# wangchou/whisper.coreml

Hardware: AMD Instinct MI355X
Metric: xRT (audio-s/s) large-v3 beam=5 @1/2/4/8 GPU; p50 per-token decode ms (higher is better)
Workload: dtype fp16; 1 GPU; large-v3 beam=5 transcribe() of one 600 s file, 30 s clip grid, condition_on_previous_text=False, temperature=0; model=large-v3, global_batch=20, seq_len=448

## Files before the change

include/whisper_hip.h:

```cpp
#ifndef WHISPER_HIP_H
#define WHISPER_HIP_H
#include <stdint.h>

#ifdef __cplusplus
extern "C" {
#endif

typedef struct wh_ctx wh_ctx;

typedef struct wh_dims {
  int n_mels, n_audio_ctx, n_audio_state, n_audio_head, n_audio_layer;
  int n_vocab, n_text_ctx, n_text_state, n_text_head, n_text_layer;
} wh_dims;

enum { WH_F32 = 0, WH_F16 = 1 };

typedef struct wh_decode_opts {
  int group;
  int beam;
  float patience;
  float temperature;
  int sample_len;
  int suppress_blank;
  int timestamps;
// ... 63 lines not shown
int wh_decode_maxc(wh_ctx* ctx);

int wh_prefill(wh_ctx* ctx, int n_win, int group, const int* tokens, const int* n_tokens, int max_tokens,
               const int* sot_index, float* logits);
int wh_step(wh_ctx* ctx, const int* tokens, const int* text_offsets, float* logits);
int wh_reorder_kv(wh_ctx* ctx, const int* source_rows);

int wh_prefill_logits(wh_ctx* ctx, int slot, const int* tokens, int n_tokens, float* logits, const int* align_heads,
                      int n_align, float* align_qk);

int wh_align(wh_ctx* ctx, int slot, const int* tokens, int n_tokens, int n_sot, int num_frames, const int* align_heads,
             int n_align, int medfilt_width, float* token_probs, int* path, int* path_len);
int wh_align_batch(wh_ctx* ctx, int n_win, const int* slots, const int* tokens, const int* n_tokens, int n_sot,
                   const int* num_frames, const int* align_heads, int n_align, int medfilt_width, float* token_probs,
                   int* paths, int* path_lens);
int wh_dtw(wh_ctx* ctx, const float* x, int n_rows, int n_cols, int* path, int* path_len);

int wh_step_kernels(wh_ctx* ctx, int n_win, int group, char* buf, int cap);

enum { WH_N_STATS = 16 };
enum {
  WH_STAT_MEL_MS = 0, WH_STAT_ENCODE_MS, WH_STAT_PREFILL_MS, WH_STAT_STEPS_MS, WH_STAT_STEPS, WH_STAT_ENCODE_WINDOWS,
  WH_STAT_INGEST_COPY_MS, WH_STAT_INGEST_KERNEL_MS, WH_STAT_FLAC_UPLOAD_MS, WH_STAT_FLAC_PARSE_MS,
  WH_STAT_FLAC_RESTORE_MS, WH_STAT_FLAC_GATHER_MS, WH_STAT_FLAC_RESAMPLE_MS, WH_STAT_FLAC_INDEX_MS,
  WH_STAT_VAD_ENERGY_MS, WH_STAT_VAD_SPANS_MS
};
int wh_stats(wh_ctx* ctx, double* out, int n);
int wh_sync(wh_ctx* ctx);

int wh_token_ms(wh_ctx* ctx, float* out, int cap, int* n, int reset);

int wh_time_stage(wh_ctx* ctx, int what, int iters, double* ms_per_iter);

int wh_flac_info(const uint8_t* data, int64_t n, int* sample_rate, int* channels, int* bits_per_sample,
                 int64_t* total_samples);
int wh_flac_decode(const uint8_t* data, int64_t n, int32_t* out, int64_t cap_frames, int64_t* n_frames);
const char* wh_flac_last_error(void);

int wh_flac_index(const uint8_t* data, int64_t n, int64_t* offsets, int32_t* fields, int64_t cap, int64_t* n_cand);
int wh_flac_decode_indexed(const uint8_t* data, int64_t n, int32_t* out, int64_t cap_frames, int64_t* n_frames);
int wh_flac_last_path(void);
int wh_flac_decode_device(wh_ctx* ctx, const uint8_t* data, int64_t n_bytes, int32_t* out, int64_t cap_frames,
                          int64_t* n_frames, int* path_out);
int wh_flac_ingest(wh_ctx* ctx, const uint8_t* data, int64_t n_bytes, int up, int down, const double* taps,
                   int n_taps, int64_t dst_offset, int64_t reserve, int64_t* n_out, int* path_out);

enum { WH_WAV_U8 = 0, WH_WAV_S16, WH_WAV_S24, WH_WAV_S32, WH_WAV_F32, WH_WAV_F64, WH_WAV_ALAW, WH_WAV_ULAW };
typedef struct wh_wav_fmt { int encoding, channels, sample_rate, valid_bits; int64_t data_offset, n_frames; } wh_wav_fmt;
int wh_wav_info(const uint8_t* data, int64_t n, wh_wav_fmt* out);
const char* wh_wav_last_error(void);
int wh_wav_ingest(wh_ctx* ctx, const uint8_t* data, int64_t n_bytes, int up, int down, const double* taps,
                  int n_taps, int64_t dst_offset, int64_t reserve, int64_t* n_out);

#ifdef __cplusplus
}
#endif
#endif
```

whisper.coreml_amd/csrc/wh_gemm.h:

```cpp
#pragma once
#include "wh_common.h"

namespace wh {

enum Epi {
  EPI_STORE = 0,
  EPI_STORE_GELU = 1,
  EPI_RESID = 2,
  EPI_GELU_POS = 3,
  EPI_HEADSPLIT = 4,
  EPI_QKV_DEC = 5,
  EPI_F32_COLS = 6,
  EPI_PARTIAL = 7,
  EPI_QKV_ENC = 8,
};

struct GemmArgs {
  const void* X = nullptr;
  const void* W = nullptr;
  const float* bias = nullptr;
  int M = 0, N = 0, K = 0;
  int ldx = 0;
  int x_group_rows = 1 << 30;
  int64_t x_group_stride = 0;
// ... 113 lines not shown
      const int m = mrow(g0 + j);
      if (m >= a.M) continue;
      const int gi = m / a.x_group_rows, ri = m - gi * a.x_group_rows;
#pragma unroll
      for (int ni = 0; ni < NI; ++ni) {
        const int n = ncol(ni);
        float4_t v = acc[g0 + j][ni];
        if (a.bias) v += bv[ni];
        if constexpr (EPI == EPI_RESID) {
          float4_t c = xv[j][ni];
          c += v;
          store4(a.out_f32 + (int64_t)m * a.ldo + n, c[0], c[1], c[2], c[3]);
        } else if constexpr (EPI == EPI_GELU_POS) {
          const float4_t p = xv[j][ni];
          store4(a.out_f32 + (int64_t)m * a.ldo + n, gelu_f(v[0]) + p[0], gelu_f(v[1]) + p[1], gelu_f(v[2]) + p[2],
                 gelu_f(v[3]) + p[3]);
        } else {
          epilogue_store<T, EPI>(a, m, gi, ri, n, v);
        }
      }
    }
  }
}

template <typename T>
int launch_gemm(const GemmArgs& a, int epi, hipStream_t st);
template <typename T>
int launch_gemm_tiles(const GemmArgs& a, int epi, int tile_sel, hipStream_t st);

template <typename T>
int launch_proj_partial(const GemmArgs& a, int max_z, hipStream_t st, int* z_out, hipEvent_t ev0 = nullptr,
                        hipEvent_t ev1 = nullptr);

bool proj1_supported(int R, int n);
template <typename T>
int launch_proj1(const GemmArgs& a, int epi, bool ln, hipStream_t st, hipEvent_t ev0 = nullptr,
                 hipEvent_t ev1 = nullptr);

int gemv_ksplit(int M, int N, int K, int max_z = 16, int mt_block = 0);

}
```

whisper.coreml_amd/csrc/wh_proj.h:

```cpp
#pragma once
#include "wh_gemm.h"

#ifndef WH_PROJ_KZ_SLOW
#define WH_PROJ_KZ_SLOW 0
#endif
#ifndef WH_PROJ_XSLOW
#define WH_PROJ_XSLOW 0
#endif

namespace wh {

template <typename T, int MT, int NSUB, int KW, int NSTEP>
struct ProjShape {
  static constexpr int CT = 16 * NSUB, MR = 16 * MT;
  static constexpr int KC = KW * NSTEP * 32;
  static constexpr int XROW = KC * (int)sizeof(T) + 16;
  static constexpr int CPR = KC * (int)sizeof(T) / 16;
  static constexpr int NT = 64 * NSUB * KW;
  static constexpr int XC = (MR * CPR + NT - 1) / NT;
  static constexpr int XBYTES = MR * XROW;
  static constexpr int RBYTES = (KW - 1) * NSUB * MT * 64 * 16;
  static constexpr int LDS = XBYTES > RBYTES ? XBYTES : RBYTES;
};

// ... 103 lines not shown
  const int n = n0 + 4 * g;
  if (n >= a.N) return;
#pragma unroll
  for (int mt = 0; mt < MT; ++mt) {
    const int m = m0 + mt * 16 + r;
    if (m >= a.M) continue;
    float4_t v = acc[mt];
    if constexpr (EPI == EPI_PARTIAL) {
#if WH_WT
      const int64_t e = ((int64_t)kz * a.M + m) * a.ldo + n;
      if (sizeof(T) == 2 && a.slab_half) {
        typedef unsigned u32x2 __attribute__((ext_vector_type(2)));
        const half4_t hv = (half4_t){(half_t)v[0], (half_t)v[1], (half_t)v[2], (half_t)v[3]};
        __builtin_amdgcn_raw_buffer_store_b64(__builtin_bit_cast(u32x2, hv), wt_rsrc(a.out_f32), (int)(e * 2), 0, 16);
      } else {
        wt_store4(wt_rsrc(a.out_f32), (int)(e * 4), v);
      }
#else
      store4(a.out_f32 + ((int64_t)kz * a.M + m) * a.ldo + n, v[0], v[1], v[2], v[3]);
#endif
    } else if constexpr (EPI == EPI_F32_COLS) {
      float* o = a.out_f32 + (int64_t)m * a.ldo;
#pragma unroll
      for (int j = 0; j < 4; ++j)
        if (n + j < a.N) o[n + j] = v[j] + (a.bias ? a.bias[n + j] : 0.f);
    } else {
      if (a.bias) v += load4f(a.bias + n);
      epilogue_store<T, EPI>(a, m, 0, m, n, v);
    }
  }
  CT_END(ct_slot);
}

constexpr int P1_RMAX = 8;

template <typename T, int NSUB, int KW, int NSTEP, int CPL>
struct Proj1Shape {
  static constexpr int KC = KW * NSTEP * 32;
  static constexpr int XROW = KC * (int)sizeof(T) + 16;
  static constexpr int XBYTES = CPL ? P1_RMAX * XROW : 0;
  static constexpr int RBYTES = (KW - 1) * NSUB * 64 * 16;
  static constexpr int LDS = (XBYTES > RBYTES ? XBYTES : RBYTES) > 16 ? (XBYTES > RBYTES ? XBYTES : RBYTES) : 16;
};

constexpr int P1_PEND = 1, P1_DEFER = 2;

template <typename T, int NSUB, int KW, int NSTEP, int ZS, int CPL, int EPI, int MODE>
__global__ __launch_bounds__(64 * NSUB * KW) void k_proj1(GemmArgs a) {
  using P = Proj1Shape<T, NSUB, KW, NSTEP, CPL>;
  constexpr bool LN = CPL > 0;
  constexpr bool PEND = LN && (MODE & P1_PEND), DEFER = (MODE & P1_DEFER) && ZS == 2 && EPI == EPI_RESID;
  constexpr int NWV = NSUB * KW;
  constexpr int RPW = (P1_RMAX + NWV - 1) / NWV;
  extern __shared__ __attribute__((aligned(16))) char xs[];
  const int tid = threadIdx.x, lane = tid & 63, wave = tid >> 6, r = lane & 15, g = lane >> 4;
  const int sub = wave % NSUB, kw = wave / NSUB;
  const int R = a.M, K = a.K, kz = blockIdx.y;
  const int tile = blockIdx.x * NSUB + sub;
  const int n0 = tile * 16;
  const int kb = kz * P::KC;
  const int kw0 = kb + kw * NSTEP * 32;
  const T* W = reinterpret_cast<const T*>(a.W);
  const int ct_slot = a.N == a.K ? CT_PROJ_NN : a.N == 3 * a.K ? CT_PROJ_QKV : a.N == 4 * a.K ? CT_PROJ_FC1 : CT_PROJ_FC2;
  CT_MARK(ct_slot, 0);

  const int CH = K / 4;
// ... 177 lines not shown
```

whisper.coreml_amd/csrc/wh_proj.hip:

```cpp
#include <array>
#include <cstdio>
#include <cstdlib>
#include <vector>

#include "wh_proj.h"
#include <hip/hip_ext.h>

namespace wh {

namespace {

struct Cfg { int nsub, kw, nstep; };
constexpr Cfg CFGS[] = {{4, 1, 5}, {4, 1, 10}, {5, 1, 10}, {4, 1, 4}, {4, 1, 6},
                        {4, 1, 20}, {5, 1, 20}, {8, 1, 5}, {8, 1, 10},
                        {4, 1, 8}};
constexpr int NCFG = sizeof(CFGS) / sizeof(CFGS[0]);
constexpr int NRANKED = NCFG - 1;

typedef void (*KFn)(GemmArgs);
struct Ent { KFn f; int lds; };

template <typename T, int MT, int C>
Ent ent() {
  constexpr Cfg c = CFGS[C];
  return {&k_proj<T, MT, c.nsub, c.kw, c.nstep, EPI_PARTIAL>, ProjShape<T, MT, c.nsub, c.kw, c.nstep>::LDS};
}
template <typename T, int MT>
void row(Ent* e) {
  e[0] = ent<T, MT, 0>(); e[1] = ent<T, MT, 1>(); e[2] = ent<T, MT, 2>(); e[3] = ent<T, MT, 3>(); e[4] = ent<T, MT, 4>();
  e[5] = ent<T, MT, 5>(); e[6] = ent<T, MT, 6>(); e[7] = ent<T, MT, 7>(); e[8] = ent<T, MT, 8>();
  e[9] = ent<T, MT, 9>();
  static_assert(NCFG == 10, "one entry per configuration");
}
template <typename T>
struct Table {
  Ent e[7][NCFG];
  bool attr[7][NCFG] = {};
  Table() {
    row<T, 1>(e[0]); row<T, 2>(e[1]); row<T, 3>(e[2]); row<T, 4>(e[3]);
    row<T, 5>(e[4]); row<T, 6>(e[5]); row<T, 7>(e[6]);
  }
};

constexpr int LDS_MAX = 160 * 1024;

}

template <typename T>
int launch_proj_partial(const GemmArgs& a, int max_z, hipStream_t st, int* z_out, hipEvent_t ev0, hipEvent_t ev1) {
  static Table<T> tab;
  static const bool off = [] {
    const char* e = tune_env("WHISPER_HIP_PROJ");
    return e && e[0] == '0';
  }();
  if (off || a.M < 1 || a.M > 112 || a.K % 32 || a.N % 16 || a.x_group_rows < a.M) return -1;
  const int mt = (a.M + 15) / 16, S = a.K / 32;
  static const std::vector<std::array<int, 3>> force = [] {
    std::vector<std::array<int, 3>> v;
    if (const char* e = tune_env("WHISPER_HIP_PROJ_FORCE")) {
      int n, k, c, off = 0, used = 0;
      while (sscanf(e + off, "%d:%d:%d%n", &n, &k, &c, &used) == 3) {
        v.push_back({n, k, c});
        off += used;
        if (e[off] == ',') ++off;
        else break;
      }
    }
    return v;
  }();
  int forced = -1;
  for (const auto& f : force)
    if (f[0] == a.N && f[1] == a.K && f[2] >= 0 && f[2] < NCFG) forced = f[2];
  int best = -1, best_wgs = 0, best_z = 0;
  for (int c = 0; c < NCFG; ++c) {
    const Cfg& k = CFGS[c];
    if (c >= NRANKED && best >= 0 && forced < 0) break;
    if (S % (k.kw * k.nstep)) continue;
    const int z = S / (k.kw * k.nstep);
    if (z > 16 || tab.e[6][c].lds > LDS_MAX) continue;
    const int wgs = (a.N + 16 * k.nsub - 1) / (16 * k.nsub) * z;
    if (forced >= 0) {
      if (c == forced) best = c, best_wgs = wgs, best_z = z;
      continue;
    }
    if (wgs > 256) continue;
    const bool deep = k.nstep >= 5;
    const bool bdeep = best >= 0 && CFGS[best].nstep >= 5;
    if (best < 0 || (deep && !bdeep) ||
        (deep == bdeep && (wgs > best_wgs || (wgs == best_wgs && k.nstep > CFGS[best].nstep))))
      best = c, best_wgs = wgs, best_z = z;
  }
  if (best < 0 || best_z > max_z) return -1;
  const Ent& e = tab.e[mt - 1][best];
  if (!tab.attr[mt - 1][best]) {
    if (hipFuncSetAttribute(reinterpret_cast<const void*>(e.f), hipFuncAttributeMaxDynamicSharedMemorySize, e.lds) !=
        hipSuccess)
      return -2;
    tab.attr[mt - 1][best] = true;
  }
  GemmArgs b = a;
  b.ksplit = best_z;
  if (ev0)
    hipExtLaunchKernelGGL(e.f, dim3(best_wgs), dim3(64 * CFGS[best].nsub * CFGS[best].kw), e.lds, st, ev0, ev1, 0, b), wh_launched("k_proj");
  else {
    hipLaunchKernelGGL(e.f, dim3(best_wgs), dim3(64 * CFGS[best].nsub * CFGS[best].kw), e.lds, st, b);
    wh_launched("k_proj");
  }
  *z_out = best_z;
  return 0;
}

namespace {
template <typename T, int NSUB, int KW, int NS, int ZS, int CPL, int EPI, int MODE = 0>
int p1_go(const GemmArgs& a, hipStream_t st, hipEvent_t ev0, hipEvent_t ev1) {
  using P = Proj1Shape<T, NSUB, KW, NS, CPL>;
  static_assert(P::LDS <= 64 * 1024, "k_proj1 LDS");
  static_assert(NSUB * KW <= 16, "k_proj1 waves");
  if (a.K != ZS * P::KC || a.N % (16 * NSUB)) return -1;
  if (ZS > 1 && (!a.p1_slab || !a.p1_cnt || (int64_t)ZS * (a.N / 16) > a.p1_slabs)) return -1;
  if ((MODE & P1_PEND) && (!a.res_slab || !a.res_bias || !a.x_out || a.x_out == a.xf32)) return -1;
  const dim3 grid(a.N / (16 * NSUB), ZS), block(64 * NSUB * KW);
  void (*f)(GemmArgs) = &k_proj1<T, NSUB, KW, NS, ZS, CPL, EPI, MODE>;
  if (ev0)
    hipExtLaunchKernelGGL(f, grid, block, P::LDS, st, ev0, ev1, 0, a), wh_launched("k_proj1");
  else {
    hipLaunchKernelGGL(f, grid, block, P::LDS, st, a);
    wh_launched("k_proj1");
  }
  return 0;
}

template <typename T, int CPL, int BKW, int NS, int F1SUB>
int p1_width_launch(const GemmArgs& a, int epi, bool ln, int n, hipStream_t st, hipEvent_t e0, hipEvent_t e1) {
  if (ln) {
    if (a.K != n) return -1;
    if (a.res_slab) {
      if (epi == EPI_QKV_DEC && a.N == 3 * n) return p1_go<T, 1, BKW, NS, 1, CPL, EPI_QKV_DEC, P1_PEND>(a, st, e0, e1);
      if (epi == EPI_STORE_GELU && a.N == 4 * n)
        return p1_go<T, F1SUB, BKW, NS, 1, CPL, EPI_STORE_GELU, P1_PEND>(a, st, e0, e1);
      if (epi == EPI_STORE && a.N == n) return p1_go<T, 1, BKW, NS, 1, CPL, EPI_STORE, P1_PEND>(a, st, e0, e1);
      return -1;
    }
    if (epi == EPI_QKV_DEC && a.N == 3 * n) return p1_go<T, 1, BKW, NS, 1, CPL, EPI_QKV_DEC>(a, st, e0, e1);
// ... 52 lines not shown
```

whisper.coreml_amd/csrc/wh_runtime.hip:

```cpp
#include <hip/hip_runtime.h>

#include <algorithm>
#include <chrono>
#include <cmath>
#include <cstdio>
#include <cstring>
#include <set>
#include <string>
#include <vector>

#include "whisper_hip.h"
#include "wh_align.h"
#include "wh_audio.h"
#include "wh_gemm.h"
#include "wh_host.h"
#include "wh_kernels.h"

using namespace wh;

static thread_local std::string g_release_error;

namespace {

constexpr int CTX = 448;
// ... 34 lines not shown
struct DecLayer {
  float *ln1_g, *ln1_b, *bqkv, *bo, *lnx_g, *lnx_b, *bqx, *box, *ln2_g, *ln2_b, *b1, *b2;
  T *wqkv, *wo, *wqx, *wox, *w1, *w2;
  T* wqx_f = nullptr;
};

}

struct wh_ctx {
  virtual std::string step_kernels(int n_win, int group) const = 0;
  virtual ~wh_ctx() {}
  virtual int load(const std::string& name, const float* data, const int64_t* shape, int ndim) = 0;
  virtual int finalize() = 0;
  virtual int encode(int n_win, const int64_t* seeks, const int* segs) = 0;
  virtual int read_xa(int slot, float* out) = 0;
  virtual int read_ckv(int slot, int layer, float* k, float* v) = 0;
  virtual int decode_begin(int n_win, const wh_decode_opts* o, const int* init, const int* n_init, int max_init,
                           const int* sot_index, const int* slots) = 0;
  virtual int decode_steps(int max_steps, int* n_done) = 0;
  virtual int step_prefill(int n_win, int G, const int* init, const int* n_init, int max_init, const int* sot_index,
                           float* lg) = 0;
  virtual int step_tokens(const int* tok, const int* offsets, float* lg) = 0;
  virtual int reorder_kv(const int* src) = 0;
  virtual int decode_read(int slot, int* tokens, float* slp, int* len, int* fin_n, int* fin_tok, int* fin_len,
                          float* fin_score, float* nsp) = 0;
  virtual int prefill_logits(int slot, const int* tokens, int n, float* logits, const int* ah, int na, float* aqk) = 0;
  virtual int align(int slot, const int* tokens, int n, int n_sot, int num_frames, const int* ah, int na, int medfilt,
                    float* probs, int* path, int* plen) = 0;
  virtual int align_batch(int n_win, const int* slots, const int* tokens, const int* n_tokens, int n_sot,
                          const int* num_frames, const int* ah, int na, int medfilt, float* probs, int* paths,
                          int* plens) = 0;
  virtual int dtw(const float* x, int N, int M, int* path, int* plen) = 0;
  virtual int time_stage(int what, int iters, double* ms) = 0;
  virtual int share_weights_from(wh_ctx* src) = 0;
  int sharers = 0;
  wh_ctx* shares_from = nullptr;
  std::vector<float> token_ms;
  double stats[WH_N_STATS] = {0};
  AudioFront audio;
  int n_mels = 0;
  int maxc = 5;
  int maxc_stride = 1;
  int device = 0;
};

namespace {

template <typename T>
struct Ctx : public wh_ctx {
  wh_dims d;
  int ns, nh, La, Ld, V, K1p;
  int Wcap, Gcap;
  hipStream_t st = nullptr;
  Arena wa;
  Arena aa;
  void* wbase = nullptr;
  void* abase = nullptr;
  std::set<std::string> loaded;
  size_t expected = 0;
  bool finalized = false;

  T *conv1_w, *conv2_w, *E, *Pdec, *ckv_w;
  float *conv1_b, *conv2_b, *pos_enc, *lnp_g, *lnp_b, *ln_g, *ln_b, *ckv_b;
  std::vector<EncLayer<T>> enc;
  std::vector<DecLayer<T>> dec;

// ... 485 lines not shown
    GemmArgs g;
    g.X = X; g.ldx = ldx; g.W = W; g.M = R; g.N = N; g.K = K; g.x_group_rows = R;
    g.out_f32 = part; g.ldo = N;
    g.slab_half = half_ok && sizeof(T) == 2 && slab16_enabled();
    slab_h = g.slab_half;
    const int maxz = part_slabs(R, N);
    const bool tev = proj_ev_n < (int)proj_ev.size() / 2;
    const int rc = tev ? launch_proj_partial<T>(g, maxz, st, ks, proj_ev[2 * proj_ev_n], proj_ev[2 * proj_ev_n + 1])
                       : launch_proj_partial<T>(g, maxz, st, ks);
    if (tev && rc == 0) ++proj_ev_n;
    if (rc == 0) return 0;
    if (rc != -1) return fail(-20, "k_proj launch failed code " + std::to_string(rc));
    slab_h = 0;
    *ks = gemv_ksplit(R, N, K, maxz);
    g = GemmArgs();
    g.out_f32 = part; g.ldo = N; g.ksplit = *ks;
    return gemm(X, ldx, W, nullptr, R, N, K, EPI_PARTIAL, g);
  }

  int resid(const T* X, int K, const T* W, const float* b, int R, const float* lg, const float* lb) {
    const int n = ns;
    GemmArgs g;
    if (R > 128) {
      g.out_f32 = x_d; g.ldo = n;
      TRY(gemm(X, K, W, b, R, n, K, EPI_RESID, g));
      launch_resid_ln<T>(x_d, nullptr, 0, 0, nullptr, xn_d, lg, lb, R, n, 1e-5f, st);
    } else {
      int ks = 0;
      TRY(partial(X, K, W, R, n, K, &ks));
      launch_resid_ln<T>(x_d, part, ks, (int64_t)R * n, b, xn_d, lg, lb, R, n, 1e-5f, st, slab_h);
    }
    return 0;
  }
  int proj(const T* W, const float* b, int R, int N, T* out, int gelu, bool skinny) {
    GemmArgs g;
    if (skinny) {
      int ks = 0;
      TRY(partial(xn_d, ns, W, R, N, ns, &ks));
      launch_reduce_store<T>(part, ks, (int64_t)R * N, b, out, N, R, N, gelu, st, slab_h);
    } else {
      g.out = out; g.ldo = N;
      TRY(gemm(xn_d, ns, W, b, R, N, ns, gelu ? EPI_STORE_GELU : EPI_STORE, g));
    }
    return 0;
  }

  int sa_probe_ks = 1;
  int sa_probe_half = 0;
  int dec_layers(int R, const int* rw, const int* rs, const int* rp, int ancG, int nwin, const int* wr0, const int* wnr,
                 const int* wsl, float* aqk, const int* qkmap, int qkrows, bool step = false,
                 const int* anc = nullptr) {
    const int* A = anc ? anc : S.anc;
    const int n = ns;
    const bool skinny = step && R <= 128;
    GemmArgs g;
    final_x = nullptr;
    if (step && !qkmap && p1_active(R, nwin))
      return dec_layers_p1(R, rw, rs, rp, ancG, nwin, wr0, wnr, wsl, A);
    launch_layernorm<T>(x_d, xn_d, dec[0].ln1_g, dec[0].ln1_b, R, n, 1e-5f, nullptr, st);
    for (int l = 0; l < Ld; ++l) {
      auto& e = dec[l];
      if (skinny) {
        int ks = 0;
        TRY(partial(xn_d, n, e.wqkv, R, 3 * n, n, &ks, slab16_qkv()));
        sa_probe_ks = ks;
        sa_probe_half = slab_h;
        if (launch_self_attn_qkv<T>(part, ks, (int64_t)R * 3 * n, e.bqkv, n, kc[l], vc[l], rw, rs, rp, A, ancG,
                                    Gcap, nh, CTX, att_d, n, R, st, slab_h))
// ... 56 lines not shown
    const int n = ns;
    auto& e = dec[l];
    if (p1_active(R, cur_nwin)) {
      GemmArgs g;
      g.W = e.wqkv; g.bias = e.bqkv; g.M = R; g.N = 3 * n; g.K = n;
      g.xf32 = x_d; g.ln_g = e.ln1_g; g.ln_b = e.ln1_b; g.ln_eps = 1e-5f;
      g.out = q_d; g.ldo = n; g.hs_state = n; g.hs_heads = nh;
      g.row_win = st_row_win; g.row_slot = st_row_slot; g.row_pos = row_pos; g.kc = kc[l]; g.vc = vc[l];
      g.kv_beams = Gcap; g.kv_ctx = CTX;
      TRY(p1(g, EPI_QKV_DEC, true));
      struct Q { const T* X; int K; const T* W; const float* b; int N; int epi; const float* lg; const float* lb; T* out; };
      const Q qs[5] = {{att_d, n, e.wo, e.bo, n, EPI_RESID, nullptr, nullptr, nullptr},
                       {nullptr, n, e.wqx, e.bqx, n, EPI_STORE, e.lnx_g, e.lnx_b, q_d},
                       {att_d, n, e.wox, e.box, n, EPI_RESID, nullptr, nullptr, nullptr},
                       {nullptr, n, e.w1, e.b1, 4 * n, EPI_STORE_GELU, e.ln2_g, e.ln2_b, hm_d},
                       {hm_d, 4 * n, e.w2, e.b2, n, EPI_RESID, nullptr, nullptr, nullptr}};
      for (const Q& q : qs) {
        g = GemmArgs();
        g.W = q.W; g.bias = q.b; g.M = R; g.N = q.N; g.K = q.K;
        if (q.lg) {
          g.xf32 = x_d; g.ln_g = q.lg; g.ln_b = q.lb; g.ln_eps = 1e-5f; g.out = q.out; g.ldo = q.N;
        } else {
          g.X = q.X; g.ldx = q.K; g.out_f32 = x_d; g.ldo = n;
        }
        TRY(p1(g, q.epi, q.lg != nullptr));
      }
      return 0;
    }
    struct P { const T* X; int K; const T* W; int N; } ps[6] = {
        {xn_d, n, e.wqkv, 3 * n}, {att_d, n, e.wo, n}, {xn_d, n, e.wqx, n},
        {att_d, n, e.wox, n},     {xn_d, n, e.w1, 4 * n}, {hm_d, 4 * n, e.w2, n}};
    for (auto& p : ps) {
      if (p.W == e.wqx && xq_proj_active(cur_G)) continue;
      int ks = 0;
      TRY(partial(p.X, p.K, p.W, R, p.N, p.K, &ks));
    }
    return 0;
  }

  bool p1_active(int R, int n_win) const { return n_win == 1 && p1_enabled() && proj1_supported(R, ns); }
  std::string step_kernels(int n_win, int group) const override {
    const bool p1 = p1_active(n_win * group, n_win), h = sizeof(T) == 2;
    return std::string("proj=") + (p1 ? "k_proj1" : "k_proj") + ",xattn=k_xattn_seg" +
           (!p1 && xq_proj_active(group) ? "<qproj>" : "") + ",self_attn=" +
           (p1 ? (h ? "k_self_attn<kco>" : "k_self_attn") : h ? "k_self_attn_qkv<pipe+kco>" : "k_self_attn_qkv") +
           ",tail=vocab+k_logit_part";
  }

  int dec_layers_p1(int R, const int* rw, const int* rs, const int* rp, int ancG, int nwin, const int* wr0,
                    const int* wnr, const int* wsl, const int* A) {
    const int n = ns;
    float* xc = x_d;
    float* xo = x2_d;
    const float* pend = nullptr;
    auto ln_in = [&](GemmArgs& g, const float* lg, const float* lb) {
      g.xf32 = xc; g.ln_g = lg; g.ln_b = lb; g.ln_eps = 1e-5f;
      if (pend) { g.res_slab = p1_slab; g.res_bias = pend; g.x_out = xo; }
    };
    auto ln_done = [&]() {
      if (pend) { std::swap(xc, xo); pend = nullptr; }
    };
    auto resid = [&](const T* X, int K, const T* W, const float* b, bool defer) -> int {
      GemmArgs g;
      g.X = X; g.ldx = K; g.W = W; g.bias = b; g.M = R; g.N = n; g.K = K; g.out_f32 = xc; g.ldo = n;
      g.p1_defer = defer;
      TRY(p1(g, EPI_RESID, false));
      if (defer) pend = b;
      return 0;
    };
    for (int l = 0; l < Ld; ++l) {
      auto& e = dec[l];
      GemmArgs g;
      g.W = e.wqkv; g.bias = e.bqkv; g.M = R; g.N = 3 * n; g.K = n;
      ln_in(g, e.ln1_g, e.ln1_b);
      g.out = q_d; g.ldo = n; g.hs_state = n; g.hs_heads = nh;
      g.row_win = rw; g.row_slot = rs; g.row_pos = rp; g.kc = kc[l]; g.vc = vc[l]; g.kv_beams = Gcap; g.kv_ctx = CTX;
      TRY(p1(g, EPI_QKV_DEC, true));
      ln_done();
      launch_self_attn<T>(q_d, n, kc[l], vc[l], rw, rs, rp, A, ancG, Gcap, nh, CTX, att_d, n, R, st);
// ... 860 lines not shown
             int n_align, int medfilt_width, float* token_probs, int* path, int* path_len) {
  CTXCALL(ctx->align(slot, tokens, n_tokens, n_sot, num_frames, align_heads, n_align, medfilt_width, token_probs, path,
                     path_len));
}
int wh_align_batch(wh_ctx* ctx, int n_win, const int* slots, const int* tokens, const int* n_tokens, int n_sot,
                   const int* num_frames, const int* align_heads, int n_align, int medfilt_width, float* token_probs,
                   int* paths, int* path_lens) {
  CTXCALL(ctx->align_batch(n_win, slots, tokens, n_tokens, n_sot, num_frames, align_heads, n_align, medfilt_width,
                           token_probs, paths, path_lens));
}
int wh_dtw(wh_ctx* ctx, const float* x, int n_rows, int n_cols, int* path, int* path_len) {
  CTXCALL(ctx->dtw(x, n_rows, n_cols, path, path_len));
}
int wh_stats(wh_ctx* ctx, double* out, int n) {
  if (!ctx || !out) return fail(-1, "null argument");
  for (int i = 0; i < n && i < WH_N_STATS; ++i) out[i] = ctx->stats[i];
  return 0;
}
int wh_step_kernels(wh_ctx* ctx, int n_win, int group, char* buf, int cap) {
  if (!ctx || !buf || cap < 1) return fail(-1, "bad arguments");
  const std::string d = ctx->step_kernels(n_win, group);
  const int n = std::min<int>((int)d.size(), cap - 1);
  memcpy(buf, d.data(), n);
  buf[n] = 0;
  return n;
}
int wh_sync(wh_ctx* ctx) {
  const int rc = enter(ctx, __func__);
  if (rc) return rc;
  HIPCHK(hipDeviceSynchronize());
  return launch_status(__func__);
}
int wh_time_stage(wh_ctx* ctx, int what, int iters, double* ms) { CTXCALL(ctx->time_stage(what, iters, ms)); }
#if WH_TUNING
int wh_tune_share_weights(wh_ctx* ctx, wh_ctx* src) {
  if (!src) return fail(-1, "null source context");
  CTXCALL(ctx->share_weights_from(src));
}
#endif

}
```

whisper.coreml_amd/whisper/backend_hip.py:

```python

import ctypes
import os
from ctypes import POINTER, c_char_p, c_double, c_float, c_int, c_int64, c_uint64, c_void_p
from typing import NamedTuple, Optional, Sequence

import numpy as np

_PKG_DIR = os.path.dirname(os.path.abspath(__file__))
_DEFAULT_LIB = os.path.join(os.path.dirname(_PKG_DIR), "lib", "libwhisper_hip.so")

WH_F32 = 0
WH_F16 = 1
WH_PCM_S16, WH_PCM_S32, WH_PCM_F32 = 0, 1, 2


class HipBackendError(RuntimeError):
    pass


class WhDims(ctypes.Structure):
    _fields_ = [(k, c_int) for k in ("n_mels", "n_audio_ctx", "n_audio_state", "n_audio_head", "n_audio_layer",
                                     "n_vocab", "n_text_ctx", "n_text_state", "n_text_head", "n_text_layer")]


# ... 42 lines not shown
                                c_int64, c_int64, POINTER(c_int64)]),
    "wh_audio_read": (c_int, [c_void_p, c_void_p, c_int64, c_int64]),
    "wh_speech_spans": (c_int, [c_void_p, POINTER(WhVadOpts), c_int, c_void_p, c_int, c_void_p, c_void_p]),
    "wh_frame_energy_read": (c_int, [c_void_p, c_int, c_void_p, c_int64, c_void_p]),
    "wh_mel_max": (c_int, [c_void_p, POINTER(c_float)]),
    "wh_mel_normalize": (c_int, [c_void_p, c_float]),
    "wh_log_mel_batch": (c_int, [c_void_p, c_void_p, c_int, c_void_p, c_int64, c_int, c_void_p]),
    "wh_mel_max_batch": (c_int, [c_void_p, c_void_p, c_int]),
    "wh_mel_read": (c_int, [c_void_p, c_void_p, c_int64, c_int64]),
    "wh_mel_write": (c_int, [c_void_p, c_void_p, c_int64]),
    "wh_encode": (c_int, [c_void_p, c_int, c_void_p, c_void_p]),
    "wh_read_audio_features": (c_int, [c_void_p, c_int, c_void_p]),
    "wh_read_cross_kv": (c_int, [c_void_p, c_int, c_int, c_void_p, c_void_p]),
    "wh_decode_begin": (c_int, [c_void_p, c_int, POINTER(WhDecodeOpts), c_void_p, c_void_p, c_int, c_void_p]),
    "wh_decode_begin_slots": (c_int, [c_void_p, c_int, c_void_p, POINTER(WhDecodeOpts), c_void_p, c_void_p, c_int,
                                      c_void_p]),
    "wh_decode_steps": (c_int, [c_void_p, c_int, POINTER(c_int)]),
    "wh_decode_read": (c_int, [c_void_p, c_int, c_void_p, c_void_p, c_void_p, c_void_p, c_void_p, c_void_p,
                               c_void_p, c_void_p]),
    "wh_decode_maxc": (c_int, [c_void_p]),
    "wh_prefill": (c_int, [c_void_p, c_int, c_int, c_void_p, c_void_p, c_int, c_void_p, c_void_p]),
    "wh_step": (c_int, [c_void_p, c_void_p, c_void_p, c_void_p]),
    "wh_reorder_kv": (c_int, [c_void_p, c_void_p]),
    "wh_prefill_logits": (c_int, [c_void_p, c_int, c_void_p, c_int, c_void_p, c_void_p, c_int, c_void_p]),
    "wh_align": (c_int, [c_void_p, c_int, c_void_p, c_int, c_int, c_int, c_void_p, c_int, c_int, c_void_p, c_void_p,
                         POINTER(c_int)]),
    "wh_align_batch": (c_int, [c_void_p, c_int, c_void_p, c_void_p, c_void_p, c_int, c_void_p, c_void_p, c_int,
                               c_int, c_void_p, c_void_p, c_void_p]),
    "wh_dtw": (c_int, [c_void_p, c_void_p, c_int, c_int, c_void_p, POINTER(c_int)]),
    "wh_stats": (c_int, [c_void_p, POINTER(c_double), c_int]),
    "wh_sync": (c_int, [c_void_p]),
    "wh_time_stage": (c_int, [c_void_p, c_int, c_int, POINTER(c_double)]),
    "wh_step_kernels": (c_int, [c_void_p, c_int, c_int, ctypes.c_char_p, c_int]),
    "wh_token_ms": (c_int, [c_void_p, c_void_p, c_int, POINTER(c_int), c_int]),
    "wh_flac_info": (c_int, [c_void_p, c_int64, POINTER(c_int), POINTER(c_int), POINTER(c_int), POINTER(c_int64)]),
    "wh_flac_decode": (c_int, [c_void_p, c_int64, c_void_p, c_int64, POINTER(c_int64)]),
    "wh_flac_last_error": (c_char_p, []),
    "wh_flac_index": (c_int, [c_void_p, c_int64, c_void_p, c_void_p, c_int64, POINTER(c_int64)]),
    "wh_flac_decode_indexed": (c_int, [c_void_p, c_int64, c_void_p, c_int64, POINTER(c_int64)]),
    "wh_flac_last_path": (c_int, []),
    "wh_flac_decode_device": (c_int, [c_void_p, c_void_p, c_int64, c_void_p, c_int64, POINTER(c_int64),
                                      POINTER(c_int)]),
    "wh_flac_ingest": (c_int, [c_void_p, c_void_p, c_int64, c_int, c_int, c_void_p, c_int, c_int64, c_int64,
                               POINTER(c_int64), POINTER(c_int)]),
    "wh_wav_info": (c_int, [c_void_p, c_int64, POINTER(WhWavFmt)]),
    "wh_wav_last_error": (c_char_p, []),
    "wh_wav_ingest": (c_int, [c_void_p, c_void_p, c_int64, c_int, c_int, c_void_p, c_int, c_int64, c_int64,
                              POINTER(c_int64)]),
}
N_STATS = 16
FLAC_PATHS = ("device", "host")


def lib_path() -> str:
    return os.environ.get("WHISPER_HIP_LIB", _DEFAULT_LIB)


def load_library(path: Optional[str] = None):
    global _lib
    if _lib is not None and path is None:
        return _lib
    p = path or lib_path()
    if not os.path.exists(p):
        raise HipBackendError(f"libwhisper_hip.so not found at {p}; build it with `make -C whisper.coreml_amd`")
    lib = ctypes.CDLL(p)
    for name, (res, args) in _EXPORTS.items():
# ... 420 lines not shown
        path = np.zeros((2, N + M), dtype=np.int32)
        n = c_int(0)
        self._check(self.lib.wh_dtw(self.h, _ptr(x), N, M, _ptr(path), ctypes.byref(n)), "wh_dtw")
        return path[:, :n.value].copy()

    def stats(self) -> dict:
        out = (c_double * N_STATS)()
        self._check(self.lib.wh_stats(self.h, out, N_STATS), "wh_stats")
        keys = ["mel_ms", "encode_ms", "prefill_ms", "steps_ms", "steps", "encode_windows", "ingest_copy_ms",
                "ingest_kernel_ms", "flac_upload_ms", "flac_parse_ms", "flac_restore_ms", "flac_gather_ms",
                "flac_resample_ms", "flac_index_ms", "vad_energy_ms", "vad_spans_ms"]
        return {k: out[i] for i, k in enumerate(keys)}

    def sync(self):
        self._check(self.lib.wh_sync(self.h), "wh_sync")

    def token_ms(self, reset: bool = False) -> np.ndarray:
        n = c_int(0)
        self._check(self.lib.wh_token_ms(self.h, None, 0, ctypes.byref(n), 0), "wh_token_ms")
        out = np.zeros(max(n.value, 1), np.float32)
        self._check(self.lib.wh_token_ms(self.h, _ptr(out), n.value, ctypes.byref(n), int(reset)), "wh_token_ms")
        return out[:n.value]

    def step_kernels(self, n_win: int, group: int) -> dict:
        buf = ctypes.create_string_buffer(256)
        n = self.lib.wh_step_kernels(self.h, n_win, group, buf, 256)
        self._check(0 if n >= 0 else n, "wh_step_kernels")
        return dict(kv.split("=", 1) for kv in buf.value.decode().split(","))

    def time_stage(self, what: int, iters: int) -> float:
        ms = c_double()
        self._check(self.lib.wh_time_stage(self.h, what, iters, ctypes.byref(ms)), "wh_time_stage")
        return ms.value
```

Measured before the change: 759.3 audio-s/s.

## Fuse decoder FC1 split-K GEMM, reduction, bias and GELU into one kernel

Adds k_fc1_whole, a single kernel for the decoder MLP up-projection. It performs the split-K partial products across waves within one workgroup, reduces them through LDS, then adds bias, applies GELU and stores fp16. This replaces the previous k_proj partial launch plus a separate reduce/store kernel, removing one launch and the global round trip of the partial slabs on every decode step. It is on by default for fp16 when the tiling picker would choose z=4 with 10 steps. It also adds a comparison API to check numerics against the old path, since the fp16 rounding of the intermediate slabs is kept.

```diff
diff --git a/include/whisper_hip.h b/include/whisper_hip.h
--- a/include/whisper_hip.h
+++ b/include/whisper_hip.h
@@ -119,6 +119,8 @@
 
 int wh_time_stage(wh_ctx* ctx, int what, int iters, double* ms_per_iter);
 
+int wh_fc1_compare(wh_ctx* ctx, int layer, int path, const float* x, int rows, float* out);
+
 int wh_flac_info(const uint8_t* data, int64_t n, int* sample_rate, int* channels, int* bits_per_sample,
                  int64_t* total_samples);
 int wh_flac_decode(const uint8_t* data, int64_t n, int32_t* out, int64_t cap_frames, int64_t* n_frames);
diff --git a/whisper.coreml_amd/csrc/wh_gemm.h b/whisper.coreml_amd/csrc/wh_gemm.h
--- a/whisper.coreml_amd/csrc/wh_gemm.h
+++ b/whisper.coreml_amd/csrc/wh_gemm.h
@@ -169,6 +169,11 @@
 int launch_proj_partial(const GemmArgs& a, int max_z, hipStream_t st, int* z_out, hipEvent_t ev0 = nullptr,
                         hipEvent_t ev1 = nullptr);
 
+template <typename T>
+bool fc1_whole_served(int M, int N, int K);
+template <typename T>
+int launch_fc1_whole(const GemmArgs& a, hipStream_t st, hipEvent_t ev0 = nullptr, hipEvent_t ev1 = nullptr);
+
 bool proj1_supported(int R, int n);
 template <typename T>
 int launch_proj1(const GemmArgs& a, int epi, bool ln, hipStream_t st, hipEvent_t ev0 = nullptr,
diff --git a/whisper.coreml_amd/csrc/wh_proj.h b/whisper.coreml_amd/csrc/wh_proj.h
--- a/whisper.coreml_amd/csrc/wh_proj.h
+++ b/whisper.coreml_amd/csrc/wh_proj.h
@@ -159,6 +159,132 @@
   CT_END(ct_slot);
 }
 
+constexpr int FC1_RG = 56;
+constexpr int FC1_RMAX = 112;
+
+template <typename T, int MT, int NSUB, int TPW, int Z, int NSTEP>
+struct Fc1Shape {
+  static constexpr int CT = 16 * NSUB * TPW;
+  static constexpr int K = Z * NSTEP * 32;
+  static constexpr int MR = 16 * MT < FC1_RG ? 16 * MT : FC1_RG;
+  static constexpr int XROW = K * (int)sizeof(T) + 16;
+  static constexpr int CPR = K * (int)sizeof(T) / 16;
+  static constexpr int NT = 64 * NSUB * Z;
+  static constexpr int XC = (MR * CPR + NT - 1) / NT;
+  static constexpr int xbytes(int rg) { return rg * XROW + 16; }
+  static constexpr int RROW = CT * 2 + 8;
+  static constexpr int RSLICE = 16 * MT * RROW;
+  static constexpr int RBYTES = Z * RSLICE;
+  static constexpr int lds(int rg) { return xbytes(rg) > RBYTES ? xbytes(rg) : RBYTES; }
+};
+
+template <typename T, int MT, int NSUB, int TPW, int Z, int NSTEP>
+__global__ __launch_bounds__(64 * NSUB * Z, (MT <= 2 && NSUB * Z <= 8) ? 2 : 1) void k_fc1_whole(GemmArgs a) {
+  static_assert(NSUB * Z <= 16, "at most 16 waves");
+  static_assert(sizeof(T) == 2, "fp16 contexts (the fp16 slab rounding is part of the result)");
+  using P = Fc1Shape<T, MT, NSUB, TPW, Z, NSTEP>;
+  constexpr int NT = P::NT;
+  extern __shared__ __attribute__((aligned(16))) char xs[];
+  const int tid = threadIdx.x, lane = tid & 63, wave = tid >> 6, r = lane & 15, g = lane >> 4;
+  const int sub = wave % NSUB, z = wave / NSUB;
+  const int nct = (a.N + P::CT - 1) / P::CT, nmg = a.row_groups;
+  const int bid = xcd_remap(blockIdx.x, nct * nmg);
+  const int mg = bid % nmg, ct = bid / nmg;
+  const int rg = (a.M + nmg - 1) / nmg, m0 = mg * rg, rows = min(rg, a.M - m0);
+  const int n0 = ct * P::CT + sub * TPW * 16;
+  CT_MARK(CT_PROJ_FC1, 0);
+
+  const char* X = reinterpret_cast<const char*>(a.X);
+  float4_t xv[P::XC];
+  constexpr int DR = NT / P::CPR, DC = NT % P::CPR;
+  const int ldx2 = a.ldx * (int)sizeof(T);
+  const auto rsx = __builtin_amdgcn_make_buffer_rsrc(const_cast<char*>(X) + (int64_t)m0 * ldx2, 0, rows * ldx2, 0x00020000);
+  {
+    int col = tid % P::CPR, off = (tid / P::CPR) * ldx2 + col * 16;
+#pragma unroll
+    for (int i = 0; i < P::XC; ++i) {
+      xv[i] = __builtin_bit_cast(float4_t, __builtin_amdgcn_raw_buffer_load_b128(rsx, off, 0, 0));
+      col += DC;
+      off += DR * ldx2 + DC * 16;
+      if (col >= P::CPR) {
+        col -= P::CPR;
+        off += ldx2 - P::CPR * 16;
+      }
+    }
+  }
+  __builtin_amdgcn_sched_barrier(0);
+  Frag<T> wf[TPW][NSTEP];
+  const T* wp[TPW];
+#pragma unroll
+  for (int t = 0; t < TPW; ++t)
+    wp[t] = reinterpret_cast<const T*>(a.W) + (int64_t)min(n0 + t * 16 + r, a.N - 1) * a.K + z * NSTEP * 32 + 8 * g;
+#pragma unroll
+  for (int s = 0; s < NSTEP; ++s)
+#pragma unroll
+    for (int t = 0; t < TPW; ++t) frag_load_stream(wf[t][s], wp[t] + s * 32);
+  constexpr int QPR = P::CT / 4;
+  constexpr bool PRE_B = NT % QPR == 0;
+  float4_t pre_b = (float4_t){0.f, 0.f, 0.f, 0.f};
+  if (PRE_B && a.bias) pre_b = load4f(a.bias + min(ct * P::CT + 4 * (tid % QPR), a.N - 4));
+  __builtin_amdgcn_sched_barrier(0);
+#pragma unroll
+  for (int i = 0; i < P::XC; ++i) {
+    const int c = tid + NT * i;
+    const int row = c / P::CPR, col = c - row * P::CPR;
+    *reinterpret_cast<float4_t*>(xs + (row < rg ? row * P::XROW + col * 16 : rg * P::XROW)) = xv[i];
+  }
+  __syncthreads();
+  CT_MARK(CT_PROJ_FC1, 1);
+
+  float4_t acc[TPW][MT];
+  const char* xl[MT];
+#pragma unroll
+  for (int mt = 0; mt < MT; ++mt) {
+#pragma unroll
+    for (int t = 0; t < TPW; ++t) acc[t][mt] = (float4_t){0.f, 0.f, 0.f, 0.f};
+    xl[mt] = xs + min(mt * 16 + r, rg - 1) * P::XROW + (z * NSTEP * 32 + 8 * g) * (int)sizeof(T);
+  }
+#pragma unroll
+  for (int s = 0; s < NSTEP; ++s) {
+#pragma unroll
+    for (int mt = 0; mt < MT; ++mt) {
+      Frag<T> xf;
+      frag_load(xf, reinterpret_cast<const T*>(xl[mt] + s * 32 * (int)sizeof(T)));
+#pragma unroll
+      for (int t = 0; t < TPW; ++t) mfma_step(acc[t][mt], wf[t][s], xf);
+    }
+  }
+  CT_MARK(CT_PROJ_FC1, 2);
+
+  __syncthreads();
+#pragma unroll
+  for (int t = 0; t < TPW; ++t)
+#pragma unroll
+    for (int mt = 0; mt < MT; ++mt) {
+      const float4_t v = acc[t][mt];
+      *reinterpret_cast<half4_t*>(xs + z * P::RSLICE + (mt * 16 + r) * P::RROW + ((sub * TPW + t) * 16 + 4 * g) * 2) =
+          (half4_t){(half_t)v[0], (half_t)v[1], (half_t)v[2], (half_t)v[3]};
+    }
+  __syncthreads();
+
+#pragma unroll
+  for (int q = tid; q < MT * 16 * QPR; q += NT) {
+    const int row = q / QPR, cq = q - row * QPR;
+    const int n = ct * P::CT + 4 * cq;
+    if (row >= rows || n >= a.N) continue;
+    float4_t v = pre_b;
+    if (!PRE_B && a.bias) v = load4f(a.bias + n);
+#pragma unroll
+    for (int s = 0; s < Z; ++s) {
+      const half4_t h = *reinterpret_cast<const half4_t*>(xs + s * P::RSLICE + row * P::RROW + cq * 8);
+      v += (float4_t){(float)h[0], (float)h[1], (float)h[2], (float)h[3]};
+    }
+    store4(reinterpret_cast<T*>(a.out) + (int64_t)(m0 + row) * a.ldo + n, gelu_f(v[0]), gelu_f(v[1]), gelu_f(v[2]),
+           gelu_f(v[3]));
+  }
+  CT_END(CT_PROJ_FC1);
+}
+
 constexpr int P1_RMAX = 8;
 
 template <typename T, int NSUB, int KW, int NSTEP, int CPL>
diff --git a/whisper.coreml_amd/csrc/wh_proj.hip b/whisper.coreml_amd/csrc/wh_proj.hip
--- a/whisper.coreml_amd/csrc/wh_proj.hip
+++ b/whisper.coreml_amd/csrc/wh_proj.hip
@@ -1,3 +1,4 @@
+#include <algorithm>
 #include <array>
 #include <cstdio>
 #include <cstdlib>
@@ -19,6 +20,7 @@
 
 typedef void (*KFn)(GemmArgs);
 struct Ent { KFn f; int lds; };
+struct Fc1Ent { KFn f; int xrow, rbytes; };
 
 template <typename T, int MT, int C>
 Ent ent() {
@@ -44,17 +46,22 @@
 
 constexpr int LDS_MAX = 160 * 1024;
 
-}
-
-template <typename T>
-int launch_proj_partial(const GemmArgs& a, int max_z, hipStream_t st, int* z_out, hipEvent_t ev0, hipEvent_t ev1) {
+template <typename T>
+Table<T>& table() {
   static Table<T> tab;
-  static const bool off = [] {
-    const char* e = tune_env("WHISPER_HIP_PROJ");
-    return e && e[0] == '0';
-  }();
-  if (off || a.M < 1 || a.M > 112 || a.K % 32 || a.N % 16 || a.x_group_rows < a.M) return -1;
-  const int mt = (a.M + 15) / 16, S = a.K / 32;
+  return tab;
+}
+
+}
+
+namespace {
+
+struct Pick { int cfg, z, wgs; };
+template <typename T>
+bool pick_tiling(int N, int K, Pick* out) {
+  const Table<T>& tab = table<T>();
+  if (K % 32 || N % 16) return false;
+  const int S = K / 32;
   static const std::vector<std::array<int, 3>> force = [] {
     std::vector<std::array<int, 3>> v;
     if (const char* e = tune_env("WHISPER_HIP_PROJ_FORCE")) {
@@ -70,7 +77,7 @@
   }();
   int forced = -1;
   for (const auto& f : force)
-    if (f[0] == a.N && f[1] == a.K && f[2] >= 0 && f[2] < NCFG) forced = f[2];
+    if (f[0] == N && f[1] == K && f[2] >= 0 && f[2] < NCFG) forced = f[2];
   int best = -1, best_wgs = 0, best_z = 0;
   for (int c = 0; c < NCFG; ++c) {
     const Cfg& k = CFGS[c];
@@ -78,7 +85,7 @@
     if (S % (k.kw * k.nstep)) continue;
     const int z = S / (k.kw * k.nstep);
     if (z > 16 || tab.e[6][c].lds > LDS_MAX) continue;
-    const int wgs = (a.N + 16 * k.nsub - 1) / (16 * k.nsub) * z;
+    const int wgs = (N + 16 * k.nsub - 1) / (16 * k.nsub) * z;
     if (forced >= 0) {
       if (c == forced) best = c, best_wgs = wgs, best_z = z;
       continue;
@@ -90,7 +97,29 @@
         (deep == bdeep && (wgs > best_wgs || (wgs == best_wgs && k.nstep > CFGS[best].nstep))))
       best = c, best_wgs = wgs, best_z = z;
   }
-  if (best < 0 || best_z > max_z) return -1;
+  if (best < 0) return false;
+  *out = {best, best_z, best_wgs};
+  return true;
+}
+
+bool proj_off() {
+  static const bool off = [] {
+    const char* e = tune_env("WHISPER_HIP_PROJ");
+    return e && e[0] == '0';
+  }();
+  return off;
+}
+
+}
+
+template <typename T>
+int launch_proj_partial(const GemmArgs& a, int max_z, hipStream_t st, int* z_out, hipEvent_t ev0, hipEvent_t ev1) {
+  Table<T>& tab = table<T>();
+  if (proj_off() || a.M < 1 || a.M > 112 || a.K % 32 || a.N % 16 || a.x_group_rows < a.M) return -1;
+  const int mt = (a.M + 15) / 16;
+  Pick pk;
+  if (!pick_tiling<T>(a.N, a.K, &pk) || pk.z > max_z) return -1;
+  const int best = pk.cfg, best_z = pk.z, best_wgs = pk.wgs;
   const Ent& e = tab.e[mt - 1][best];
   if (!tab.attr[mt - 1][best]) {
     if (hipFuncSetAttribute(reinterpret_cast<const void*>(e.f), hipFuncAttributeMaxDynamicSharedMemorySize, e.lds) !=
@@ -109,6 +138,94 @@
   *z_out = best_z;
   return 0;
 }
+
+namespace {
+constexpr int FC1_Z = 4, FC1_NSTEP = 10;
+struct Fc1Cfg { int nsub, tpw; };
+constexpr int FC1_WIDE = 0, FC1_NARROW = 1;
+#if WH_TUNING
+constexpr Fc1Cfg FC1_CFGS[] = {{2, 2}, {1, 2}, {4, 1}, {3, 1}, {2, 1}, {1, 3}, {1, 4}, {2, 3}};
+#else
+constexpr Fc1Cfg FC1_CFGS[] = {{2, 2}, {1, 2}};
+#endif
+constexpr int FC1_WIDE_GROUPS = 3;
+constexpr int FC1_NN = sizeof(FC1_CFGS) / sizeof(FC1_CFGS[0]);
+constexpr int FC1_NMAX = 8;
+
+template <int MT, int I>
+Fc1Ent fc1_ent() {
+  constexpr Fc1Cfg c = FC1_CFGS[I < FC1_NN ? I : 0];
+  using P = Fc1Shape<half_t, MT, c.nsub, c.tpw, FC1_Z, FC1_NSTEP>;
+  static_assert(P::lds(P::MR) <= LDS_MAX, "k_fc1_whole LDS");
+  return {&k_fc1_whole<half_t, MT, c.nsub, c.tpw, FC1_Z, FC1_NSTEP>, P::XROW, P::RBYTES};
+}
+template <int MT>
+void fc1_row(Fc1Ent* e) {
+  e[0] = fc1_ent<MT, 0>(); e[1] = fc1_ent<MT, 1>(); e[2] = fc1_ent<MT, 2>(); e[3] = fc1_ent<MT, 3>();
+  e[4] = fc1_ent<MT, 4>(); e[5] = fc1_ent<MT, 5>(); e[6] = fc1_ent<MT, 6>(); e[7] = fc1_ent<MT, 7>();
+  static_assert(FC1_NN <= FC1_NMAX, "one entry per configuration");
+}
+struct Fc1Table {
+  Fc1Ent e[4][FC1_NMAX];
+  int attr[4][FC1_NMAX] = {};
+  Fc1Table() { fc1_row<1>(e[0]); fc1_row<2>(e[1]); fc1_row<3>(e[2]); fc1_row<4>(e[3]); }
+};
+}
+
+template <typename T>
+bool fc1_whole_served(int M, int N, int K) {
+  if constexpr (sizeof(T) != 2) return false;
+  if (proj_off() || M < 1 || M > FC1_RMAX || N != 4 * K) return false;
+  Pick pk;
+  if (!pick_tiling<T>(N, K, &pk)) return false;
+  return pk.z == FC1_Z && CFGS[pk.cfg].kw * CFGS[pk.cfg].nstep == FC1_NSTEP;
+}
+
+template <typename T>
+int launch_fc1_whole(const GemmArgs& a, hipStream_t st, hipEvent_t ev0, hipEvent_t ev1) {
+  if constexpr (sizeof(T) != 2) {
+    return -1;
+  } else {
+    static Fc1Table tab;
+    if (!fc1_whole_served<T>(a.M, a.N, a.K) || a.ldx != a.K || a.x_rows || a.x_group_rows < a.M || !a.out || a.ldo < a.N)
+      return -1;
+    int sel = a.M > FC1_RG ? FC1_WIDE : FC1_NARROW;
+    if (const char* e = tune_env("WHISPER_HIP_FC1_CFG"))
+      if (atoi(e) >= 0 && atoi(e) < FC1_NN) sel = atoi(e);
+    const int nsub = FC1_CFGS[sel].nsub, ctw = 16 * nsub * FC1_CFGS[sel].tpw;
+    GemmArgs b = a;
+    const int min_groups = (a.M + FC1_RG - 1) / FC1_RG;
+    b.row_groups = a.M > FC1_RG ? FC1_WIDE_GROUPS : 1;
+    if (const char* e = tune_env("WHISPER_HIP_FC1_NMG")) {
+      const int g = atoi(e);
+      if (g >= min_groups && g <= a.M && (g - 1) * ((a.M + g - 1) / g) < a.M) b.row_groups = g;
+    }
+    const int rg = (a.M + b.row_groups - 1) / b.row_groups, mt = (rg + 15) / 16;
+    const Fc1Ent& e = tab.e[mt - 1][sel];
+    const int lds = std::max(rg * e.xrow + 16, e.rbytes);
+    if (lds > LDS_MAX) return -1;
+    if (tab.attr[mt - 1][sel] < lds) {
+      if (hipFuncSetAttribute(reinterpret_cast<const void*>(e.f), hipFuncAttributeMaxDynamicSharedMemorySize, lds) !=
+          hipSuccess)
+        return -2;
+      tab.attr[mt - 1][sel] = lds;
+    }
+    const int wgs = (a.N + ctw - 1) / ctw * b.row_groups;
+    const dim3 grid(wgs), block(64 * nsub * FC1_Z);
+    if (ev0)
+      hipExtLaunchKernelGGL(e.f, grid, block, lds, st, ev0, ev1, 0, b), wh_launched("k_fc1_whole");
+    else {
+      hipLaunchKernelGGL(e.f, grid, block, lds, st, b);
+      wh_launched("k_fc1_whole");
+    }
+    return 0;
+  }
+}
+
+template bool fc1_whole_served<float>(int, int, int);
+template bool fc1_whole_served<half_t>(int, int, int);
+template int launch_fc1_whole<float>(const GemmArgs&, hipStream_t, hipEvent_t, hipEvent_t);
+template int launch_fc1_whole<half_t>(const GemmArgs&, hipStream_t, hipEvent_t, hipEvent_t);
 
 namespace {
 template <typename T, int NSUB, int KW, int NS, int ZS, int CPL, int EPI, int MODE = 0>
diff --git a/whisper.coreml_amd/csrc/wh_runtime.hip b/whisper.coreml_amd/csrc/wh_runtime.hip
--- a/whisper.coreml_amd/csrc/wh_runtime.hip
+++ b/whisper.coreml_amd/csrc/wh_runtime.hip
@@ -90,6 +90,7 @@
                           int* plens) = 0;
   virtual int dtw(const float* x, int N, int M, int* path, int* plen) = 0;
   virtual int time_stage(int what, int iters, double* ms) = 0;
+  virtual int fc1_compare(int layer, int path, const float* x, int rows, float* out) = 0;
   virtual int share_weights_from(wh_ctx* src) = 0;
   int sharers = 0;
   wh_ctx* shares_from = nullptr;
@@ -641,8 +642,28 @@
     }
     return 0;
   }
+  static constexpr int FC1_WHOLE_MIN_ROWS = 1;
+  static int fc1_whole_min_rows() {
+    const char* off = tune_env("WHISPER_HIP_FC1_WHOLE");
+    if (off && off[0] == '0') return 1 << 30;
+    const char* e = tune_env("WHISPER_HIP_FC1_MIN_ROWS");
+    return e ? atoi(e) : FC1_WHOLE_MIN_ROWS;
+  }
+  bool fc1_whole_shape(int R, int N) const { return sizeof(T) == 2 && slab16_enabled() && fc1_whole_served<T>(R, N, ns); }
+  bool fc1_whole_active(int R, int N) const { return R >= fc1_whole_min_rows() && fc1_whole_shape(R, N); }
+  int fc1_whole(const T* W, const float* b, int R, int N, T* out) {
+    GemmArgs g;
+    g.X = xn_d; g.ldx = ns; g.W = W; g.bias = b; g.M = R; g.N = N; g.K = ns; g.x_group_rows = R;
+    g.out = out; g.ldo = N;
+    const bool tev = proj_ev_n < (int)proj_ev.size() / 2;
+    const int rc = tev ? launch_fc1_whole<T>(g, st, proj_ev[2 * proj_ev_n], proj_ev[2 * proj_ev_n + 1])
+                       : launch_fc1_whole<T>(g, st);
+    if (tev && rc == 0) ++proj_ev_n;
+    return rc == 0 ? 0 : fail(-20, "k_fc1_whole launch failed code " + std::to_string(rc));
+  }
   int proj(const T* W, const float* b, int R, int N, T* out, int gelu, bool skinny) {
     GemmArgs g;
+    if (skinny && gelu && fc1_whole_active(R, N)) return fc1_whole(W, b, R, N, out);
     if (skinny) {
       int ks = 0;
       TRY(partial(xn_d, ns, W, R, N, ns, &ks));
@@ -765,6 +786,10 @@
         {att_d, n, e.wox, n},     {xn_d, n, e.w1, 4 * n}, {hm_d, 4 * n, e.w2, n}};
     for (auto& p : ps) {
       if (p.W == e.wqx && xq_proj_active(cur_G)) continue;
+      if (p.W == e.w1 && fc1_whole_active(R, p.N)) {
+        TRY(fc1_whole(e.w1, e.b1, R, p.N, hm_d));
+        continue;
+      }
       int ks = 0;
       TRY(partial(p.X, p.K, p.W, R, p.N, p.K, &ks));
     }
@@ -777,7 +802,34 @@
     return std::string("proj=") + (p1 ? "k_proj1" : "k_proj") + ",xattn=k_xattn_seg" +
            (!p1 && xq_proj_active(group) ? "<qproj>" : "") + ",self_attn=" +
            (p1 ? (h ? "k_self_attn<kco>" : "k_self_attn") : h ? "k_self_attn_qkv<pipe+kco>" : "k_self_attn_qkv") +
-           ",tail=vocab+k_logit_part";
+           ",tail=vocab+k_logit_part" +
+           (p1 ? "" : fc1_whole_active(n_win * group, 4 * ns) ? ",fc1=k_fc1_whole" : ",fc1=k_proj+k_reduce_store");
+  }
+
+  int fc1_compare(int layer, int path, const float* x, int rows, float* out) override {
+    if (!finalized) return fail(-9, "weights not finalized");
+    if (layer < 0 || layer >= Ld || rows < 1 || rows > 128 || (path != 0 && path != 1) || !x || !out)
+      return fail(-15, "fc1_compare: bad layer, row count (1..128) or path (0, 1)");
+    if (cur_nwin >= 1 && !step_api)
+      for (int w = 0; w < cur_nwin; ++w) TRY(check_slot_idle(win_slots[w]));
+    rows_dirty = true;
+    const int n = ns, N = 4 * ns;
+    auto& e = dec[layer];
+    std::vector<T> hx((size_t)rows * n), hy((size_t)rows * N);
+    for (size_t i = 0; i < hx.size(); ++i) hx[i] = (T)x[i];
+    HIPCHK(hipMemcpyAsync(xn_d, hx.data(), hx.size() * sizeof(T), hipMemcpyHostToDevice, st));
+    if (path == 1 && fc1_whole_shape(rows, N)) {
+      TRY(fc1_whole(e.w1, e.b1, rows, N, hm_d));
+    } else {
+      int ks = 0;
+      TRY(partial(xn_d, n, e.w1, rows, N, n, &ks));
+      launch_reduce_store<T>(part, ks, (int64_t)rows * N, e.b1, hm_d, N, rows, N, 1, st, slab_h);
+    }
+    HIPCHK(hipMemcpyAsync(hy.data(), hm_d, hy.size() * sizeof(T), hipMemcpyDeviceToHost, st));
+    HIPCHK(hipStreamSynchronize(st));
+    TRY(launch_status(__func__));
+    for (size_t i = 0; i < hy.size(); ++i) out[i] = (float)hy[i];
+    return 0;
   }
 
   int dec_layers_p1(int R, const int* rw, const int* rs, const int* rp, int ancG, int nwin, const int* wr0,
@@ -1704,6 +1756,9 @@
   return launch_status(__func__);
 }
 int wh_time_stage(wh_ctx* ctx, int what, int iters, double* ms) { CTXCALL(ctx->time_stage(what, iters, ms)); }
+int wh_fc1_compare(wh_ctx* ctx, int layer, int path, const float* x, int rows, float* out) {
+  CTXCALL(ctx->fc1_compare(layer, path, x, rows, out));
+}
 #if WH_TUNING
 int wh_tune_share_weights(wh_ctx* ctx, wh_ctx* src) {
   if (!src) return fail(-1, "null source context");
diff --git a/whisper.coreml_amd/whisper/backend_hip.py b/whisper.coreml_amd/whisper/backend_hip.py
--- a/whisper.coreml_amd/whisper/backend_hip.py
+++ b/whisper.coreml_amd/whisper/backend_hip.py
@@ -98,6 +98,7 @@
     "wh_sync": (c_int, [c_void_p]),
     "wh_time_stage": (c_int, [c_void_p, c_int, c_int, POINTER(c_double)]),
     "wh_step_kernels": (c_int, [c_void_p, c_int, c_int, ctypes.c_char_p, c_int]),
+    "wh_fc1_compare": (c_int, [c_void_p, c_int, c_int, c_void_p, c_int, c_void_p]),
     "wh_token_ms": (c_int, [c_void_p, c_void_p, c_int, POINTER(c_int), c_int]),
     "wh_flac_info": (c_int, [c_void_p, c_int64, POINTER(c_int), POINTER(c_int), POINTER(c_int), POINTER(c_int64)]),
     "wh_flac_decode": (c_int, [c_void_p, c_int64, c_void_p, c_int64, POINTER(c_int64)]),
@@ -584,3 +585,11 @@
         ms = c_double()
         self._check(self.lib.wh_time_stage(self.h, what, iters, ctypes.byref(ms)), "wh_time_stage")
         return ms.value
+
+    def fc1_compare(self, layer: int, path: int, x: np.ndarray) -> np.ndarray:
+        x = np.ascontiguousarray(x, dtype=np.float32)
+        rows, n = x.shape
+        assert n == self.dims["n_text_state"]
+        out = np.empty((rows, 4 * n), dtype=np.float32)
+        self._check(self.lib.wh_fc1_compare(self.h, layer, path, _ptr(x), rows, _ptr(out)), "wh_fc1_compare")
+        return out
```

Result: no change. 760.5 audio-s/s, median of 6 (+0.1%).
